# ErlerPhilipp/points2surf

Hardware: AMD Instinct MI355X
Metric: SDF queries/sec/GPU (p2s_max, 256^3 grid) (higher is better)
Workload: dtype f32

## Files before the change

### points2surf_amd/csrc/p2s_api.hip

```cpp
#include "p2s_common.h"
#include "p2s_internal.h"
#include <vector>
#include <cstring>
#include <algorithm>
#include <mutex>
#include <cstdlib>

static thread_local char g_err[512] = "";

void p2s_set_error(const char *fmt, ...) {
    va_list ap;
    va_start(ap, fmt);
    vsnprintf(g_err, sizeof(g_err), fmt, ap);
    va_end(ap);
}

namespace {
struct DevScratch {
    std::mutex mu;
    void *p = nullptr;
    size_t cap = 0;
};
DevScratch g_scratch[P2S_MAX_DEVICES];
}

P2sScratchLock::P2sScratchLock(int device) : dev_(device) {
    if (dev_ >= 0 && dev_ < P2S_MAX_DEVICES) g_scratch[dev_].mu.lock();
}
P2sScratchLock::~P2sScratchLock() {
    if (dev_ >= 0 && dev_ < P2S_MAX_DEVICES) g_scratch[dev_].mu.unlock();
}
void *P2sScratchLock::get(size_t bytes) {
    if (dev_ < 0 || dev_ >= P2S_MAX_DEVICES) return nullptr;
    DevScratch &sl = g_scratch[dev_];
    if (bytes <= sl.cap) return sl.p;
    if (sl.p) (void)hipFree(sl.p);
    sl.p = nullptr;
    sl.cap = 0;
    const size_t want = bytes + bytes / 8;
    if (hipMalloc(&sl.p, want) != hipSuccess) {
        (void)hipGetLastError();
        sl.p = nullptr;
        return nullptr;
    }
    sl.cap = want;
    return sl.p;
}

static int screen_init(p2s_model_s *m) {
    if (m->cfg.encoder_bf16 != 0) return P2S_OK;
    const char *dense = getenv("P2S_CONV3_DENSE");
    if (dense && atoi(dense) != 0) return P2S_OK;
    DevBuf<int> flag;
    const bool ok = p2s_alloc_all(m->scr_w3h, (size_t)4 * P2S_SCR_PIECE, m->scr_mu, (size_t)4 * 1024, m->scr_counters, 3, flag, 1) &&
                    hipMemset(m->scr_counters.get(), 0, 3 * 8) == hipSuccess && hipMemset(flag.get(), 0, 4) == hipSuccess;
    int rc = P2S_OK, h = 0;
    if (!ok) {
        (void)hipGetLastError();
        p2s_set_error("allocation of the screen operands of conv3 failed");
        rc = P2S_ENOMEM;
    }
    for (int i = 0; i < 4 && rc == P2S_OK; ++i) {
        const P2sLayer layer = i < 2 ? L_S3 : L_M3;
        rc = p2s_launch_screen_prepare(m->w32(layer, i & 1), const_cast<unsigned short *>(m->screen_w(layer, i & 1)),
                                       const_cast<float *>(m->screen_mu(layer, i & 1)), nullptr, flag.get());
    }
    if (rc == P2S_OK && hipMemcpy(&h, flag.get(), 4, hipMemcpyDeviceToHost) != hipSuccess) {
        p2s_set_error("hipMemcpy(conv3 range flag) failed");
        rc = P2S_EHIP;
    }
    if (rc == P2S_OK && h) {
        m->scr_w3h.reset();
        m->scr_mu.reset();
    }
    m->stem_reuse = rc == P2S_OK && m->scr_w3h && !m->cfg.sym_sum && !m->cfg.stem_recompute;
    m->stem_max_bytes = (size_t)(m->cfg.stem_reuse_max_mb > 0 ? m->cfg.stem_reuse_max_mb : 3072) << 20;
    return rc;
}

static int model_init(p2s_model_s *m, const float *blob_host, size_t n_floats) {
    const p2s_model_cfg &cfg = m->cfg;
    if (!m->blob.alloc(n_floats)) {
        p2s_set_error("allocation of the weights failed");
        return P2S_ENOMEM;
    }
    const hipError_t e = hipMemcpy(m->blob.get(), blob_host, n_floats * sizeof(float), hipMemcpyHostToDevice);
    if (e != hipSuccess) {
        p2s_set_error("hipMemcpy(weights) failed: %s", hipGetErrorString(e));
        return P2S_EHIP;
    }
    const Precision prec = p2s_precision(cfg);
    {
        const int rc = screen_init(m);
        if (rc) return rc;
    }
    if (!prec.pieces) return P2S_OK;
    struct Item { P2sLayer layer; int z; };
    std::vector<Item> items;
    for (int kind = LK_ENC; kind < LK_FP32; ++kind) {
        if (!p2s_kind_packed((P2sLayerKind)kind, cfg)) continue;
        const int slices = kind == LK_ENC || kind == LK_ENC_HEAD ? 2 : 1;
        for (int z = 0; z < slices; ++z)
            for (int l = 0; l < P2S_LAYERS; ++l) {
                if (p2s_layers[l].kind != kind) continue;
                m->h_off[l][z] = m->h_off[l][1] = m->h_total;
                items.push_back({(P2sLayer)l, z});
                m->h_total += (size_t)p2s_layers[l].K * p2s_layers[l].N;
            }
    }
    if (!m->blob_h.alloc(m->h_total * prec.pieces)) {
        p2s_set_error("allocation of the 16-bit weights failed");
        return P2S_ENOMEM;
    }
    DevBuf<int> wflag;
    if (prec.f16 && (!wflag.alloc(1) || hipMemset(wflag.get(), 0, 4) != hipSuccess)) {
        (void)hipGetLastError();
        p2s_set_error("allocation of the weight range flag failed");
        return P2S_ENOMEM;
    }
    for (int piece = 0; piece < prec.pieces; ++piece)
        for (const Item &it : items) {
            const P2sLayerDesc &d = p2s_layers[it.layer];
            const int rc = p2s_launch_pack_bf16(m->w32(it.layer, it.z), m->blob_h.get() + (size_t)piece * m->h_total + m->h_off[it.layer][it.z],
                                                d.K, d.N, 0, 0, 1, piece, prec.f16, nullptr, wflag.get());
            if (rc) return rc;
        }
    if (prec.f16) {
        int h = 0;
        const hipError_t e2 = hipMemcpy(&h, wflag.get(), 4, hipMemcpyDeviceToHost);
        if (e2 != hipSuccess) {
            p2s_set_error("hipMemcpy(weight range flag) failed: %s", hipGetErrorString(e2));
            return P2S_EHIP;
        }
        if (h) {
            p2s_set_error("fp16 pair encoder (encoder_bf16 = 4): a BatchNorm-folded weight of this checkpoint does not fit the half "
                          "range (|w| > 6e4, or non-finite) -- use encoder_bf16 = 3 (the same accuracy) or 0 for this model");
            return P2S_EINVAL;
        }
        p2s_model_s::Fallback &fb = m->fb;
        fb.cap = 16384;
        const size_t k3 = (size_t)cfg.points_per_patch * 3, n3 = (size_t)cfg.sub_sample_size * 3, cap = fb.cap;
        const bool ok = p2s_alloc_all(fb.flags, (size_t)m->max_chunk, fb.count, 1, fb.patch, cap * k3, fb.sub, cap * n3, fb.query, cap * 3,
                                      fb.radius, cap, fb.index, cap, fb.sdf, cap, fb.logits, cap * 2) &&
                        hipMemset(fb.flags.get(), 0, (size_t)m->max_chunk * 4) == hipSuccess && hipMemset(fb.count.get(), 0, 4) == hipSuccess &&
                        hipMemset(fb.radius.get(), 0, cap * 4) == hipSuccess;
        if (!ok) {
            (void)hipGetLastError();
            p2s_set_error("allocation of the fp32 fallback buffers of the fp16 pair mode failed");
            return P2S_ENOMEM;
        }
    }
    P2S_HIP_CHECK(hipDeviceSynchronize());
    return P2S_OK;
}

extern "C" {

int p2s_abi_version(void) { return P2S_ABI_VERSION; }
const char *p2s_last_error(void) { return g_err; }

int p2s_device_count(void) {
    int n = 0;
    if (hipGetDeviceCount(&n) != hipSuccess) {
        (void)hipGetLastError();
        return 0;
    }
    return n;
}

int p2s_release_scratch(int device) {
    if (device < 0 || device >= P2S_MAX_DEVICES || device >= p2s_device_count()) {
        p2s_set_error("p2s_release_scratch: no HIP device %d", device);
        return P2S_ENODEVICE;
    }
    P2S_HIP_CHECK(hipSetDevice(device));
    {
        std::lock_guard<std::mutex> g(g_scratch[device].mu);
        if (g_scratch[device].p) (void)hipFree(g_scratch[device].p);
        g_scratch[device].p = nullptr;
        g_scratch[device].cap = 0;
    }
    p2s_cloud_pool_release(device);
    return P2S_OK;
}

int p2s_model_create(const p2s_model_cfg *cfg, const float *blob_host, size_t n_floats,
                     const p2s_weight_offsets *offs, int device, p2s_model_t *out) {
    if (!cfg || !blob_host || !offs || !out || n_floats == 0) {
        p2s_set_error("p2s_model_create: null argument");
        return P2S_EINVAL;
    }
    if (cfg->net_size != 1024 || (cfg->output_dim != 2 && cfg->output_dim != 1) || cfg->points_per_patch < 1 || cfg->sub_sample_size < 1) {
        p2s_set_error("p2s_model_create: unsupported cfg (net_size=%d output_dim=%d)", cfg->net_size, cfg->output_dim);
        return P2S_EINVAL;
    }
    if (p2s_device_count() <= device || device < 0) {
        p2s_set_error("p2s_model_create: no HIP device %d", device);
        return P2S_ENODEVICE;
    }
    if (cfg->encoder_bf16 < 0 || cfg->encoder_bf16 > 4) {
        p2s_set_error("p2s_model_create: encoder_bf16 = %d (0 fp32, 1 bf16, 2 / 3 split bf16, 4 fp16 pair)", cfg->encoder_bf16);
        return P2S_EINVAL;
    }
    P2S_HIP_CHECK(hipSetDevice(device));
    p2s_model_s *m = new p2s_model_s(*cfg, *offs, device);
    const int rc = model_init(m, blob_host, n_floats);
    if (rc) p2s_model_destroy(m);
    else *out = m;
    return rc;
}

int p2s_model_destroy(p2s_model_t m) {
    if (!m) return P2S_OK;
    (void)hipSetDevice(m->device);
    delete m;
    return P2S_OK;
}

int p2s_set_profiling(p2s_model_t m, int enabled) {
    if (!m) return P2S_EINVAL;
    m->profiling = enabled != 0;
    return P2S_OK;
}

int p2s_get_counters(p2s_model_t m, p2s_counters *out) {
    if (!m || !out) return P2S_EINVAL;
    *out = m->counters;
    if (m->scr_counters) {
        unsigned long long h[3] = {};
        P2S_HIP_CHECK(hipSetDevice(m->device));
        P2S_HIP_CHECK(hipMemcpy(h, m->scr_counters.get(), sizeof(h), hipMemcpyDeviceToHost));
        out->conv3_confirmed = (int64_t)h[0];
        out->conv3_items_dense = (int64_t)h[1];
        out->conv3_items = (int64_t)h[2];
    }
    return P2S_OK;
}

}

int p2s_prof_mark(p2s_model_s *m, hipStream_t s) {
    if (!m->profiling) return -1;
    if (m->ev_used >= (int)m->evpool.size()) {
        DevEvent e;
        if (!e.create()) return -1;
        m->evpool.push_back(std::move(e));
    }
    const int i = m->ev_used++;
    if (hipEventRecord(m->evpool[i].get(), s) != hipSuccess) return -1;
    return i;
}

void p2s_prof_span(p2s_model_s *m, int stage, int a, int b) {
    if (a >= 0 && b >= 0) m->spans.push_back({stage, a, b});
}

static void prof_reset(p2s_model_s *m) {
    m->ev_used = 0;
    m->spans.clear();
    memset(&m->counters, 0, sizeof(m->counters));
}

static void prof_collect(p2s_model_s *m) {
    if (!m->profiling || m->ev_used == 0) return;
    (void)hipEventSynchronize(m->evpool[m->ev_used - 1].get());
    for (const auto &sp : m->spans) {
        float ms = 0.f;
        if (hipEventElapsedTime(&ms, m->evpool[sp.a].get(), m->evpool[sp.b].get()) != hipSuccess) {
            (void)hipGetLastError();
            continue;
        }
        double *dst = nullptr;
        switch (sp.stage) {
            case ST_CHAIN_STN: dst = &m->counters.ms_chain_stn; break;
            case ST_HEAD: dst = &m->counters.ms_stn_head; break;
            case ST_CHAIN_MAIN: dst = &m->counters.ms_chain_main; break;
            case ST_DECODER: dst = &m->counters.ms_decoder; break;
            case ST_KNN: dst = &m->counters.ms_knn; break;
            case ST_SUB: dst = &m->counters.ms_subsample; break;
            case ST_GRID: dst = &m->counters.ms_grid; break;
            case ST_CHAIN_QSTN: dst = &m->counters.ms_chain_qstn; break;
        }
        if (dst) *dst += ms;
    }
    m->ev_used = 0;
    m->spans.clear();
}

ModelCall::ModelCall(p2s_model_s *m_, hipStream_t s_, bool pipeline_) : m(m_), s(s_), pipeline(pipeline_) {
    if (!m) return;
    if (pipeline) {
        logits = m->logits_capture;
        logits_room = m->logits_capacity;
        m->logits_capture = nullptr;
        m->logits_capacity = 0;
    }
    rc = [&]() -> int {
        P2S_HIP_CHECK(hipSetDevice(m->device));
        prof_reset(m);
        if (m->scr_counters) P2S_HIP_CHECK(hipMemsetAsync(m->scr_counters.get(), 0, 3 * 8, s));
        if (m->fb.count) {
            P2S_HIP_CHECK(hipMemsetAsync(m->fb.count.get(), 0, 4, s));
            P2S_HIP_CHECK(hipMemsetAsync(m->fb.flags.get(), 0, (size_t)m->max_chunk * 4, s));
        }
        return P2S_OK;
    }();
}

int ModelCall::fail(int code) {
    if (!m) return code;
    (void)hipStreamSynchronize(s);
    if (pipeline && m->aux) (void)hipStreamSynchronize(m->aux.get());
    if (pipeline && m->ball) (void)hipStreamSynchronize(m->ball.get());
    return code;
}

int ModelCall::finish(float *logits_out, float *sdf_out, int64_t nq) {
    m->counters.queries += nq;
    const int rc2 = p2s_fallback_finish(m, logits_out, sdf_out, s);
    if (rc2) return fail(rc2);
    prof_collect(m);
    return P2S_OK;
}

static int run_batched(p2s_model_s *m, const float *patch, const float *sub, const float *query, const float *radius,
                       int B, float *logits, float *sdf, float *fl, float *fg, hipStream_t s) {
    ModelCall call(m, s, false);
    if (!m || B < 0 || !patch || !sub || !query) {
        p2s_set_error("encode: null argument");
        return call.fail(P2S_EINVAL);
    }
    if (sdf && !radius) {
        p2s_set_error("encode: sdf_out requested without radius");
        return call.fail(P2S_EINVAL);
    }
    const int chunk = std::min(B, m->max_chunk);
    int rc = call.rc ? call.rc : p2s_model_reserve(m, chunk);
    if (rc) return call.fail(rc);
    const int PL = m->cfg.points_per_patch, PG = m->cfg.sub_sample_size;
    for (int q0 = 0; q0 < B; q0 += chunk) {
        const int C = std::min(chunk, B - q0);
        rc = p2s_run_chunk(m, p2s_precision(m->cfg), patch + (size_t)q0 * PL * 3, sub + (size_t)q0 * PG * 3, query + (size_t)q0 * 3,
                           radius ? radius + q0 : nullptr, C, logits ? logits + (size_t)q0 * m->cfg.output_dim : nullptr,
                           sdf ? sdf + q0 : nullptr, fl ? fl + (size_t)q0 * 1024 : nullptr,
                           fg ? fg + (size_t)q0 * 1024 : nullptr, s, q0);
        if (rc) return call.fail(rc);
    }
    return call.finish(logits, sdf, B);
}

extern "C" {

int p2s_encode_decode(p2s_model_t m, const float *patch_ps_dev, const float *sub_ms_dev, const float *query_dev,
                      const float *radius_dev, int B, float *logits_out_dev, float *sdf_out_dev, void *stream) {
    if (!logits_out_dev && !sdf_out_dev) {
        p2s_set_error("p2s_encode_decode: no output requested");
        return P2S_EINVAL;
    }
    return run_batched(m, patch_ps_dev, sub_ms_dev, query_dev, radius_dev, B, logits_out_dev, sdf_out_dev, nullptr,
                       nullptr, (hipStream_t)stream);
}

int p2s_encode_features(p2s_model_t m, const float *patch_ps_dev, const float *sub_ms_dev, const float *query_dev,
                        int B, float *feat_local_dev, float *feat_global_dev, void *stream) {
    if (!feat_local_dev && !feat_global_dev) {
        p2s_set_error("p2s_encode_features: no output requested");
        return P2S_EINVAL;
    }
    return run_batched(m, patch_ps_dev, sub_ms_dev, query_dev, nullptr, B, nullptr, nullptr, feat_local_dev,
                       feat_global_dev, (hipStream_t)stream);
}

}
```

### points2surf_amd/csrc/p2s_chain.hip

```cpp
#include "p2s_common.h"
#include <cstdlib>
#include <atomic>

namespace {

constexpr int MT = 64;
constexpr int SA = 68;
constexpr int SB = 132;

__device__ __forceinline__ f32x16 mfma32(float a, float b, f32x16 c) {
    return __builtin_amdgcn_mfma_f32_32x32x2f32(a, b, c, 0, 0, 0);
}

__device__ __forceinline__ f32x4 ldg4(const float *p) { return *reinterpret_cast<const f32x4 *>(p); }
__device__ __forceinline__ f32x4 lds4(const float *p) { return *reinterpret_cast<const f32x4 *>(p); }
typedef unsigned u32x4s __attribute__((ext_vector_type(4)));
__device__ __forceinline__ f32x4 bufld4(__amdgpu_buffer_rsrc_t rsrc, int voff, int soff) {
    typedef unsigned u32x4 __attribute__((ext_vector_type(4)));
    const u32x4 v = __builtin_amdgcn_raw_buffer_load_b128(rsrc, voff, soff, 0);
    f32x4 r;
    r[0] = __uint_as_float(v[0]); r[1] = __uint_as_float(v[1]); r[2] = __uint_as_float(v[2]); r[3] = __uint_as_float(v[3]);
    return r;
}

__device__ __forceinline__ void store_tile_bias_relu(const f32x16 &acc, float *dst, int stride, int row0,
                                                     int col0, float b, int lane) {
    const int col = col0 + (lane & 31);
    const int rbase = row0 + 4 * (lane >> 5);
#pragma unroll
    for (int reg = 0; reg < 16; ++reg) {
        const int row = rbase + (reg & 3) + 8 * (reg >> 2);
        dst[row * stride + col] = fmaxf(acc[reg] + b, 0.0f);
    }
}

__device__ __forceinline__ void store_tile_bias_relu(const f32x16 &acc, float *dst, int stride, int row0,
                                                     int col0, const float *__restrict__ bias, int lane) {
    store_tile_bias_relu(acc, dst, stride, row0, col0, bias[col0 + (lane & 31)], lane);
}

__device__ __forceinline__ f32x16 zero16() {
    f32x16 z;
#pragma unroll
    for (int i = 0; i < 16; ++i) z[i] = 0.0f;
    return z;
}

struct B8 {
    f32x4 v[8];
};
__device__ __forceinline__ void load_b8(B8 &b, __amdgpu_buffer_rsrc_t rsrc, int lane16, int soff) {
#pragma unroll
    for (int kg = 0; kg < 8; ++kg) b.v[kg] = bufld4(rsrc, lane16, soff + kg * 1024);
}

template <int RT, bool NEXT>
__device__ __forceinline__ void layer_k64(const float *src, int ss, int row0, B8 &b, int lane, f32x16 (&acc)[RT],
                                          __amdgpu_buffer_rsrc_t nrs, int lane16, int nsoff) {
    const float *ap = src + (row0 + (lane & 31)) * ss + 4 * (lane >> 5);
    f32x4 a[RT], na[RT];
#pragma unroll
    for (int r = 0; r < RT; ++r) a[r] = lds4(ap + 32 * r * ss);
#pragma unroll
    for (int kg = 0; kg < 8; ++kg) {
        if (kg < 7) {
#pragma unroll
            for (int r = 0; r < RT; ++r) na[r] = lds4(ap + 32 * r * ss + 8 * (kg + 1));
        }
        __builtin_amdgcn_sched_barrier(0);
#pragma unroll
        for (int t = 0; t < 4; ++t)
#pragma unroll
            for (int r = 0; r < RT; ++r)
                acc[r] = (kg == 0 && t == 0) ? mfma32(a[r][0], b.v[0][0], zero16()) : mfma32(a[r][t], b.v[kg][t], acc[r]);
        if constexpr (NEXT) b.v[kg] = bufld4(nrs, lane16, nsoff + kg * 1024);
        __builtin_amdgcn_sched_barrier(0);
        if (kg < 7) {
#pragma unroll
            for (int r = 0; r < RT; ++r) {
                __builtin_amdgcn_sched_group_barrier(0x008, 2, 0);
                __builtin_amdgcn_sched_group_barrier(0x100, 1, 0);
                __builtin_amdgcn_sched_group_barrier(0x008, 2, 0);
            }
#pragma unroll
            for (int r = 0; r < RT; ++r) a[r] = na[r];
        }
    }
}

template <int RT>
__device__ __forceinline__ void layer_k64(const float *src, int ss, int row0, B8 &b, int lane, f32x16 (&acc)[RT]) {
    layer_k64<RT, false>(src, ss, row0, b, lane, acc, __builtin_amdgcn_make_buffer_rsrc((float *)nullptr, 0, 0, 0x00020000), 0, 0);
}

template <int NT>
__device__ __forceinline__ void layer_k64_store(const float *src, int ss, int row0, const B8 &b, int lane, f32x16 &acc,
                                                __amdgpu_buffer_rsrc_t out, int lane16, int soff) {
    const float *ap = src + (row0 + (lane & 31)) * ss + 4 * (lane >> 5);
    f32x4 a = lds4(ap), na;
#pragma unroll
    for (int kg = 0; kg < 8; ++kg) {
        if (kg < 7) na = lds4(ap + 8 * (kg + 1));
        if ((kg >> 2) == NT) {
            const u32x4s v = {__float_as_uint(a[0]), __float_as_uint(a[1]), __float_as_uint(a[2]), __float_as_uint(a[3])};
            __builtin_amdgcn_raw_buffer_store_b128(v, out, lane16, soff + kg * 1024, 0);
        }
#pragma unroll
        for (int t = 0; t < 4; ++t) acc = (kg == 0 && t == 0) ? mfma32(a[0], b.v[0][0], zero16()) : mfma32(a[t], b.v[kg][t], acc);
        if (kg < 7) {
            __builtin_amdgcn_sched_group_barrier(0x008, 2, 0);
            __builtin_amdgcn_sched_group_barrier(0x100, 1, 0);
            if ((kg >> 2) == NT) {
                __builtin_amdgcn_sched_group_barrier(0x008, 1, 0);
                __builtin_amdgcn_sched_group_barrier(0x040, 1, 0);
                __builtin_amdgcn_sched_group_barrier(0x008, 1, 0);
            } else {
                __builtin_amdgcn_sched_group_barrier(0x008, 2, 0);
            }
            a = na;
        }
    }
}
__device__ __forceinline__ void layer_k64_regs(const B8 &a, B8 &b, f32x16 &acc, __amdgpu_buffer_rsrc_t nrs, int lane16, int nsoff) {
#pragma unroll
    for (int kg = 0; kg < 8; ++kg) {
#pragma unroll
        for (int t = 0; t < 4; ++t) acc = (kg == 0 && t == 0) ? mfma32(a.v[0][0], b.v[0][0], zero16()) : mfma32(a.v[kg][t], b.v[kg][t], acc);
        b.v[kg] = bufld4(nrs, lane16, nsoff + kg * 1024);
        __builtin_amdgcn_sched_barrier(0);
    }
}

__device__ __forceinline__ float tile_colmax(const f32x16 &a, const f32x16 &b) {
    float m;
    asm volatile("s_nop 15\n\ts_nop 4\n\tv_max_f32 %0, %1, %2" : "=v"(m) : "v"(a[0]), "v"(b[0]));
#pragma unroll
    for (int i = 1; i < 16; ++i) asm volatile("v_max3_f32 %0, %0, %1, %2" : "+v"(m) : "v"(a[i]), "v"(b[i]));
    return m;
}

__device__ __forceinline__ float half_max(float m) {
    const unsigned u = __float_as_uint(m);
    const auto r = __builtin_amdgcn_permlane32_swap(u, u, false, false);
    float x = __uint_as_float(r[0]), y = __uint_as_float(r[1]), o;
    asm volatile("v_max_f32 %0, %1, %2" : "=v"(o) : "v"(x), "v"(y));
    return o;
}

__device__ __forceinline__ f32x16 mfma16b(float a, float b, f32x16 c) {
    return __builtin_amdgcn_mfma_f32_16x16x1f32(a, b, c, 0, 0, 0);
}
template <bool TAIL>
__device__ __forceinline__ f32x16 mfma_r1(float a, float b, f32x16 c) {
    if constexpr (TAIL) return mfma16b(a, b, c);
    else return mfma32(a, b, c);
}
__device__ __forceinline__ float tile_colmax1(const f32x16 &a) {
    float m;
    asm volatile("s_nop 15\n\ts_nop 4\n\tv_max_f32 %0, %1, %2" : "=v"(m) : "v"(a[0]), "v"(a[1]));
#pragma unroll
    for (int i = 2; i < 16; i += 2) asm volatile("v_max3_f32 %0, %0, %1, %2" : "+v"(m) : "v"(a[i]), "v"(a[i + 1]));
    return m;
}
__device__ __forceinline__ float tail_colmax(const f32x16 &c) {
    float sa[4], sb[4];
#pragma unroll
    for (int i = 0; i < 4; ++i) {
        sa[i] = c[i] + c[8 + i];
        sb[i] = c[4 + i] + c[12 + i];
    }
    float ma, mb;
    asm volatile("v_max3_f32 %0, %1, %2, %3" : "=v"(ma) : "v"(sa[0]), "v"(sa[1]), "v"(sa[2]));
    asm volatile("v_max_f32 %0, %0, %1" : "+v"(ma) : "v"(sa[3]));
    asm volatile("v_max3_f32 %0, %1, %2, %3" : "=v"(mb) : "v"(sb[0]), "v"(sb[1]), "v"(sb[2]));
    asm volatile("v_max_f32 %0, %0, %1" : "+v"(mb) : "v"(sb[3]));
    const auto r = __builtin_amdgcn_permlane16_swap(__float_as_uint(ma), __float_as_uint(mb), false, false);
    float x = __uint_as_float(r[0]), y = __uint_as_float(r[1]), o;
    asm volatile("v_max_f32 %0, %1, %2" : "=v"(o) : "v"(x), "v"(y));
    return o;
}

__device__ __forceinline__ float tile_colsum(const f32x16 &a, const f32x16 &b, int nvalid, int lane) {
    float s = 0.0f;
    if (nvalid >= 64) {
#pragma unroll
        for (int i = 0; i < 16; ++i) s += a[i];
#pragma unroll
        for (int i = 0; i < 16; ++i) s += b[i];
    } else {
        const int r0 = 4 * (lane >> 5);
#pragma unroll
        for (int i = 0; i < 16; ++i) {
            const int r = r0 + (i & 3) + 8 * (i >> 2);
            s += (r < nvalid) ? a[i] : 0.0f;
            s += (r + 32 < nvalid) ? b[i] : 0.0f;
        }
    }
    return s;
}
__device__ __forceinline__ float half_sum(float m) {
    const unsigned u = __float_as_uint(m);
    const auto r = __builtin_amdgcn_permlane32_swap(u, u, false, false);
    return __uint_as_float(r[0]) + __uint_as_float(r[1]);
}

typedef unsigned int u32x4 __attribute__((ext_vector_type(4)));
typedef _Float16 f16x8 __attribute__((ext_vector_type(8)));
typedef _Float16 f16x2 __attribute__((ext_vector_type(2)));
typedef float f32x2 __attribute__((ext_vector_type(2)));
constexpr int SCR_HB = 128 + 8;
constexpr int SCR_QCAP = 256;
constexpr float P2S_SCR_KAPPA = 0x1.1p-10f;
constexpr int SCR_OFF_E = MT * SA + MT * SB;
constexpr int SCR_OFF_Q = SCR_OFF_E + 1024;
constexpr int SCR_OFF_RED = SCR_OFF_Q + 4 * SCR_QCAP;
constexpr int SCR_OFF_R = SCR_OFF_RED + 8;
constexpr int SCR_OFF_MU = SCR_OFF_R + 1024;
constexpr int SCR_OFF_W0 = SCR_OFF_MU + 1024;
constexpr int SCR_LDS_FLOATS = SCR_OFF_W0 + 256;
static_assert(MT * SCR_HB * 2 <= MT * SA * 4, "the fp16 copy fits the 64-channel tile it lies over");
static_assert(2 * SCR_LDS_FLOATS * 4 <= 160 * 1024, "two workgroups per CU");

__device__ __forceinline__ u32x4 scr_bufld(__amdgpu_buffer_rsrc_t rsrc, int voff, int soff) {
    return __builtin_amdgcn_raw_buffer_load_b128(rsrc, voff, soff, 0);
}
__device__ __forceinline__ u32x4 scr_lds_a(const unsigned short *buf, int row0, int kb, int lane) {
    return *reinterpret_cast<const u32x4 *>(buf + (row0 + (lane & 31)) * SCR_HB + 16 * kb + 8 * (lane >> 5));
}
__device__ __forceinline__ f32x16 scr_mfma(u32x4 a, u32x4 b, f32x16 c) {
    return __builtin_amdgcn_mfma_f32_32x32x16_f16(__builtin_bit_cast(f16x8, a), __builtin_bit_cast(f16x8, b), c, 0, 0, 0);
}
__device__ __forceinline__ unsigned scr_half2(float a, float b) {
    const f32x2 v = {a, b};
    return __builtin_bit_cast(unsigned, __builtin_convertvector(v, f16x2));
}
constexpr int SCR_CDEPTH = 4;
static_assert(16 % SCR_CDEPTH == 0, "whole passes");
template <bool SPLIT>
__device__ __forceinline__ void scr_confirm(unsigned entry, const float *hB, __amdgpu_buffer_rsrc_t w3rsrc, int wave, unsigned *E) {
    const int row = (int)(entry >> 16), cw = (int)(entry & 0xffffu);
    const int c = 256 * wave + cw;
    const float *hrow = hB + row * SB;
    const int wcol = ((c >> 5) * (16 * 64) + (c & 31)) * 16;
    float s0 = 0.0f, s1 = 0.0f;
#pragma unroll 1
    for (int g0 = 0; g0 < 16; g0 += SCR_CDEPTH) {
        f32x4 wa[SCR_CDEPTH], wb[SCR_CDEPTH];
#pragma unroll
        for (int j = 0; j < SCR_CDEPTH; ++j) {
            wa[j] = bufld4(w3rsrc, wcol + j * 1024, g0 * 1024);
            wb[j] = bufld4(w3rsrc, wcol + j * 1024 + 512, g0 * 1024);
        }
        __builtin_amdgcn_sched_barrier(0);
        const float *hh = hrow + 8 * g0;
#pragma unroll
        for (int j = 0; j < SCR_CDEPTH; ++j) {
            const f32x4 ha = lds4(hh + 8 * j), hb = lds4(hh + 8 * j + 4);
#pragma unroll
            for (int t = 0; t < 4; ++t) {
                s0 = fmaf(ha[t], wa[j][t], s0);
                if constexpr (SPLIT) s1 = fmaf(hb[t], wb[j][t], s1);
                else s0 = fmaf(hb[t], wb[j][t], s0);
            }
        }
    }
    const float s = SPLIT ? s0 + s1 : s0;
    const int bits = (int)__float_as_uint(s);
    if (bits >= 0) atomicMax(reinterpret_cast<int *>(E + cw), bits);
    else atomicMin(E + cw, (unsigned)bits);
}

template <bool SUM, bool SCREEN = false>
__global__ __launch_bounds__(256, SCREEN ? 2 : 3) void p2s_chain_kernel(ChainArgs args) {
    constexpr bool STEM_SAVE = false, STEM_LOAD = false;
#include "p2s_chain_body.inl"
}
__global__ __launch_bounds__(256, 2) void p2s_chain_save_kernel(ChainArgs args) {
    constexpr bool SUM = false, SCREEN = true, STEM_SAVE = true, STEM_LOAD = false;
#include "p2s_chain_body.inl"
}
__global__ __launch_bounds__(256, 2) void p2s_chain_reuse_kernel(ChainArgs args) {
    constexpr bool SUM = false, SCREEN = true, STEM_SAVE = false, STEM_LOAD = true;
#include "p2s_chain_body.inl"
}

__global__ __launch_bounds__(256) void p2s_fold_kernel(FoldArgs args) {
    const int tid = threadIdx.x;
    const int lane = tid & 63;
    const int wave = __builtin_amdgcn_readfirstlane(tid >> 6);
    const int e = blockIdx.y;
    const int item = blockIdx.x;
    const float *__restrict__ T = args.T[e] + (long long)item * 4096;
    const float *__restrict__ wp = args.m1t[e];
    float *__restrict__ out = args.out[e] + (long long)item * 4096;
    const int jt = wave >> 1, ot = wave & 1;
    const int kk = lane >> 5;
    f32x16 acc = zero16();
#pragma unroll
    for (int kg = 0; kg < 8; ++kg) {
        const f32x4 b = ldg4(wp + ((ot * 8 + kg) * 64 + lane) * 4);
#pragma unroll
        for (int t = 0; t < 4; ++t) {
            const float a = T[(8 * kg + 4 * kk + t) * 64 + 32 * jt + (lane & 31)];
            acc = mfma32(a, b[t], acc);
        }
    }
    unsigned short *outh = args.outh[e];
    if (outh) {
        outh += (long long)item * 4096;
#pragma unroll
        for (int g = 0; g < 4; ++g) {
            const int kg = 4 * jt + g;
            unsigned short *dst = outh + ((ot * 4 + (kg >> 1)) * 64 + (kg & 1) * 32 + (lane & 31)) * 8 + 4 * kk;
            float x[4] = {acc[4 * g + 0], acc[4 * g + 1], acc[4 * g + 2], acc[4 * g + 3]};
            if (args.f16 && args.bad_items &&
                (p2s_f16_out_of_range(x[0]) || p2s_f16_out_of_range(x[1]) || p2s_f16_out_of_range(x[2]) || p2s_f16_out_of_range(x[3])))
                args.bad_items[item] = 1;
            for (int q = 0; q < args.ns; ++q) {
                unsigned short h[4];
#pragma unroll
                for (int t = 0; t < 4; ++t) {
                    if (args.f16) {
                        const _Float16 h0 = (_Float16)x[t];
                        h[t] = __builtin_bit_cast(unsigned short, h0);
                        x[t] = (x[t] - (float)h0) * 2048.0f;
                    } else {
                        unsigned u = __float_as_uint(x[t]);
                        u += 0x7fffu + ((u >> 16) & 1u);
                        h[t] = (unsigned short)(u >> 16);
                        x[t] -= __uint_as_float((unsigned)h[t] << 16);
                    }
                }
                uint2 pk;
                pk.x = (unsigned)h[0] | ((unsigned)h[1] << 16);
                pk.y = (unsigned)h[2] | ((unsigned)h[3] << 16);
                *reinterpret_cast<uint2 *>(dst + (long long)q * args.h_piece_stride) = pk;
            }
        }
        return;
    }
#pragma unroll
    for (int g = 0; g < 4; ++g) {
        f32x4 v = {acc[4 * g + 0], acc[4 * g + 1], acc[4 * g + 2], acc[4 * g + 3]};
        *reinterpret_cast<f32x4 *>(out + ((ot * 8 + 4 * jt + g) * 64 + lane) * 4) = v;
    }
}

}

int p2s_launch_chain(const ChainArgs &args_in, hipStream_t stream) {
    const int n = args_in.br[0].n_items + args_in.br[1].n_items;
    if (n <= 0) return P2S_OK;
    ChainArgs args = args_in;
    constexpr int padlds = 0;
#ifdef P2S_DEV_ABLATE
    args.ablate = P2S_DEV_ABLATE + 0;
#endif
    const bool sum = args.br[0].pool_sum || (args.br[1].n_items > 0 && args.br[1].pool_sum);
    if (args.screen) {
        if (sum || args.br[0].short_chain || (args.br[1].n_items > 0 && args.br[1].short_chain) || !args.w3h[0] || !args.w3mu[0] ||
            (args.br[1].n_items > 0 && (!args.w3h[1] || !args.w3mu[1]))) {
            p2s_set_error("p2s_launch_chain: the screened conv3 takes full-chain max-pool passes with their screen operands");
            return P2S_EINVAL;
        }
        const int which = args.br[0].stem_in ? 2 : args.br[0].stem_out ? 1 : 0;
        for (int b = 0; b < 2; ++b) {
            const ChainBranch &br = args.br[b];
            if (br.n_items > 0 && ((br.stem_in ? 2 : br.stem_out ? 1 : 0) != which || (br.stem_in && br.stem_out) || (which && !br.stem_bad))) {
                p2s_set_error("p2s_launch_chain: the saved stem is written, or read, by both branches of a launch, with their flags");
                return P2S_EINVAL;
            }
        }
        if (which && args.br[1].n_items <= 0) {
            p2s_set_error("p2s_launch_chain: the saved stem belongs to launches of both branches");
            return P2S_EINVAL;
        }
        static std::atomic<bool> lds_set[3][P2S_MAX_DEVICES];
        const void *kernel = which == 2 ? (const void *)p2s_chain_reuse_kernel : which == 1 ? (const void *)p2s_chain_save_kernel
                                                                                            : (const void *)p2s_chain_kernel<false, true>;
        int dev = 0;
        P2S_HIP_CHECK(hipGetDevice(&dev));
        if (dev < 0 || dev >= P2S_MAX_DEVICES || !lds_set[which][dev].load()) {
            const hipError_t attr = hipFuncSetAttribute(kernel, hipFuncAttributeMaxDynamicSharedMemorySize, SCR_LDS_FLOATS * 4);
            if (attr != hipSuccess) {
                p2s_set_error("p2s_launch_chain: %d bytes of LDS for the screened conv3 refused: %s", SCR_LDS_FLOATS * 4, hipGetErrorString(attr));
                return P2S_EHIP;
            }
            if (dev >= 0 && dev < P2S_MAX_DEVICES) lds_set[which][dev].store(true);
        }
        if (which == 2) hipLaunchKernelGGL(p2s_chain_reuse_kernel, dim3(n), dim3(256), SCR_LDS_FLOATS * 4, stream, args);
        else if (which == 1) hipLaunchKernelGGL(p2s_chain_save_kernel, dim3(n), dim3(256), SCR_LDS_FLOATS * 4, stream, args);
        else hipLaunchKernelGGL((p2s_chain_kernel<false, true>), dim3(n), dim3(256), SCR_LDS_FLOATS * 4, stream, args);
    } else if (args.br[0].stem_in || args.br[0].stem_out || args.br[1].stem_in || args.br[1].stem_out) {
        p2s_set_error("p2s_launch_chain: only the screened conv3 saves or reuses the stem");
        return P2S_EINVAL;
    } else if (sum)
        hipLaunchKernelGGL(p2s_chain_kernel<true>, dim3(n), dim3(256), padlds, stream, args);
    else
        hipLaunchKernelGGL(p2s_chain_kernel<false>, dim3(n), dim3(256), padlds, stream, args);
    P2S_LAUNCH_CHECK("p2s_chain_kernel");
    return P2S_OK;
}

__global__ void p2s_screen_mu_kernel(const float *__restrict__ w3, float *__restrict__ mu) {
    const int c = blockIdx.x * blockDim.x + threadIdx.x;
    if (c >= 1024) return;
    double ss = 0.0;
    for (int g = 0; g < 16; ++g)
        for (int u = 0; u < 8; ++u) {
            const double w = w3[(((long long)(c >> 5) * 16 + g) * 64 + (u >> 2) * 32 + (c & 31)) * 4 + (u & 3)];
            ss += w * w;
        }
    const float norm = (float)(sqrt(ss) * (1.0 + 0x1p-20));
    mu[c] = 2.0f * P2S_SCR_KAPPA * (norm * (1.0f + 0x1p-10f) + 0x1p-10f);
}

int p2s_launch_screen_prepare(const float *w32, unsigned short *dst, float *mu, hipStream_t stream, int *range_flag) {
    const int rc = p2s_launch_pack_bf16(w32, dst, 128, 1024, 0, 0, 1, 0, 1, stream, range_flag);
    if (rc) return rc;
    hipLaunchKernelGGL(p2s_screen_mu_kernel, dim3(4), dim3(256), 0, stream, w32, mu);
    P2S_LAUNCH_CHECK("p2s_screen_mu_kernel");
    return P2S_OK;
}

int p2s_launch_fold(const FoldArgs &args, hipStream_t stream) {
    if (args.n_items <= 0) return P2S_OK;
    hipLaunchKernelGGL(p2s_fold_kernel, dim3(args.n_items, 2), dim3(256), 0, stream, args);
    P2S_LAUNCH_CHECK("p2s_fold_kernel");
    return P2S_OK;
}
```

Baseline: 481,200.

## Add persistent 512-thread split kernel for stem-reuse screened conv3 chain

Adds a persistent kernel with one 512-thread block per CU for the stem-reuse screened chain pass. It claims work items through extra device counters, which grow from 3 to 5, and uses an LDS layout with queue and mailbox regions, so the work can be split across more waves per item. The aim is better CU utilisation and load balance than one 256-thread block per item. It also adds an optional debug LDS-padding knob, and the new kernel body lives in an include file not shown here.

```diff
diff --git a/points2surf_amd/csrc/p2s_api.hip b/points2surf_amd/csrc/p2s_api.hip
--- a/points2surf_amd/csrc/p2s_api.hip
+++ b/points2surf_amd/csrc/p2s_api.hip
@@ -52,8 +52,8 @@
     const char *dense = getenv("P2S_CONV3_DENSE");
     if (dense && atoi(dense) != 0) return P2S_OK;
     DevBuf<int> flag;
-    const bool ok = p2s_alloc_all(m->scr_w3h, (size_t)4 * P2S_SCR_PIECE, m->scr_mu, (size_t)4 * 1024, m->scr_counters, 3, flag, 1) &&
-                    hipMemset(m->scr_counters.get(), 0, 3 * 8) == hipSuccess && hipMemset(flag.get(), 0, 4) == hipSuccess;
+    const bool ok = p2s_alloc_all(m->scr_w3h, (size_t)4 * P2S_SCR_PIECE, m->scr_mu, (size_t)4 * 1024, m->scr_counters, 5, flag, 1) &&
+                    hipMemset(m->scr_counters.get(), 0, 5 * 8) == hipSuccess && hipMemset(flag.get(), 0, 4) == hipSuccess;
     int rc = P2S_OK, h = 0;
     if (!ok) {
         (void)hipGetLastError();
@@ -298,7 +298,7 @@
     rc = [&]() -> int {
         P2S_HIP_CHECK(hipSetDevice(m->device));
         prof_reset(m);
-        if (m->scr_counters) P2S_HIP_CHECK(hipMemsetAsync(m->scr_counters.get(), 0, 3 * 8, s));
+        if (m->scr_counters) P2S_HIP_CHECK(hipMemsetAsync(m->scr_counters.get(), 0, 5 * 8, s));
         if (m->fb.count) {
             P2S_HIP_CHECK(hipMemsetAsync(m->fb.count.get(), 0, 4, s));
             P2S_HIP_CHECK(hipMemsetAsync(m->fb.flags.get(), 0, (size_t)m->max_chunk * 4, s));
diff --git a/points2surf_amd/csrc/p2s_chain.hip b/points2surf_amd/csrc/p2s_chain.hip
--- a/points2surf_amd/csrc/p2s_chain.hip
+++ b/points2surf_amd/csrc/p2s_chain.hip
@@ -284,6 +284,21 @@
 #include "p2s_chain_body.inl"
 }
 
+constexpr int SPL_OFF_F32 = 0;
+constexpr int SPL_OFF_H16 = SPL_OFF_F32 + 2 * MT * SB;
+constexpr int SPL_OFF_A = SPL_OFF_H16 + 2 * (MT * SCR_HB / 2);
+constexpr int SPL_OFF_E = SPL_OFF_A + MT * SA;
+constexpr int SPL_OFF_Q = SPL_OFF_E + 1024;
+constexpr int SPL_OFF_R = SPL_OFF_Q + 4 * SCR_QCAP;
+constexpr int SPL_OFF_MU = SPL_OFF_R + 1024;
+constexpr int SPL_OFF_HDR = SPL_OFF_MU + 1024;
+constexpr int SPL_OFF_MAIL = SPL_OFF_HDR + 16;
+constexpr int SPL_LDS_FLOATS = SPL_OFF_MAIL + 8;
+static_assert(SPL_LDS_FLOATS * 4 <= 160 * 1024 && SPL_OFF_H16 % 4 == 0 && SPL_OFF_A % 4 == 0 && (MT * SCR_HB / 2) % 4 == 0, "fits a CU, 16-byte rows");
+__global__ __launch_bounds__(512, 1) void p2s_chain_main_split_kernel(ChainArgs args) {
+#include "p2s_chain_split.inl"
+}
+
 __global__ __launch_bounds__(256) void p2s_fold_kernel(FoldArgs args) {
     const int tid = threadIdx.x;
     const int lane = tid & 63;
@@ -353,6 +368,12 @@
     if (n <= 0) return P2S_OK;
     ChainArgs args = args_in;
     constexpr int padlds = 0;
+#ifdef P2S_DEV_LDS_PAD
+    constexpr int scr_lds = SCR_LDS_FLOATS * 4 + (P2S_DEV_LDS_PAD + 0);
+    static_assert(scr_lds <= 160 * 1024, "the padded request fits a CU");
+#else
+    constexpr int scr_lds = SCR_LDS_FLOATS * 4;
+#endif
 #ifdef P2S_DEV_ABLATE
     args.ablate = P2S_DEV_ABLATE + 0;
 #endif
@@ -381,16 +402,37 @@
         int dev = 0;
         P2S_HIP_CHECK(hipGetDevice(&dev));
         if (dev < 0 || dev >= P2S_MAX_DEVICES || !lds_set[which][dev].load()) {
-            const hipError_t attr = hipFuncSetAttribute(kernel, hipFuncAttributeMaxDynamicSharedMemorySize, SCR_LDS_FLOATS * 4);
+            const hipError_t attr = hipFuncSetAttribute(kernel, hipFuncAttributeMaxDynamicSharedMemorySize, scr_lds);
             if (attr != hipSuccess) {
-                p2s_set_error("p2s_launch_chain: %d bytes of LDS for the screened conv3 refused: %s", SCR_LDS_FLOATS * 4, hipGetErrorString(attr));
+                p2s_set_error("p2s_launch_chain: %d bytes of LDS for the screened conv3 refused: %s", scr_lds, hipGetErrorString(attr));
                 return P2S_EHIP;
             }
             if (dev >= 0 && dev < P2S_MAX_DEVICES) lds_set[which][dev].store(true);
         }
-        if (which == 2) hipLaunchKernelGGL(p2s_chain_reuse_kernel, dim3(n), dim3(256), SCR_LDS_FLOATS * 4, stream, args);
-        else if (which == 1) hipLaunchKernelGGL(p2s_chain_save_kernel, dim3(n), dim3(256), SCR_LDS_FLOATS * 4, stream, args);
-        else hipLaunchKernelGGL((p2s_chain_kernel<false, true>), dim3(n), dim3(256), SCR_LDS_FLOATS * 4, stream, args);
+#if !defined(P2S_DEV_ABLATE) && !defined(P2S_DEV_LDS_PAD)
+        if (which == 2 && args.scr_counters && dev >= 0 && dev < P2S_MAX_DEVICES) {
+            static std::atomic<int> split_cus[P2S_MAX_DEVICES];
+            int cus = split_cus[dev].load();
+            if (cus == 0) {
+                int count = 0;
+                P2S_HIP_CHECK(hipDeviceGetAttribute(&count, hipDeviceAttributeMultiprocessorCount, dev));
+                if (hipFuncSetAttribute((const void *)p2s_chain_main_split_kernel, hipFuncAttributeMaxDynamicSharedMemorySize,
+                                        SPL_LDS_FLOATS * 4) != hipSuccess) {
+                    (void)hipGetLastError();
+                    count = -1;
+                }
+                split_cus[dev].store(cus = count > 0 ? count : -1);
+            }
+            if (cus > 0) {
+                hipLaunchKernelGGL(p2s_chain_main_split_kernel, dim3(n < cus ? n : cus), dim3(512), SPL_LDS_FLOATS * 4, stream, args);
+                P2S_LAUNCH_CHECK("p2s_chain_main_split_kernel");
+                return P2S_OK;
+            }
+        }
+#endif
+        if (which == 2) hipLaunchKernelGGL(p2s_chain_reuse_kernel, dim3(n), dim3(256), scr_lds, stream, args);
+        else if (which == 1) hipLaunchKernelGGL(p2s_chain_save_kernel, dim3(n), dim3(256), scr_lds, stream, args);
+        else hipLaunchKernelGGL((p2s_chain_kernel<false, true>), dim3(n), dim3(256), scr_lds, stream, args);
     } else if (args.br[0].stem_in || args.br[0].stem_out || args.br[1].stem_in || args.br[1].stem_out) {
         p2s_set_error("p2s_launch_chain: only the screened conv3 saves or reuses the stem");
         return P2S_EINVAL;
```

New measurement: 428,900. 0.891x the previous value.
